# mataiyuan/ASD-SLAM

Hardware: AMD Instinct MI355X
Metric: frames/sec end-to-end tracking+LocalBA, KITTI 00 mono @2000 keypoints (higher is better)
Workload: dtype f32

## Files before the change

asd-slam_amd/csrc/asdnet.hip:

```cpp
#include "ctx.h"

#include <algorithm>
#include <cmath>
#include <cstring>

typedef float f32x16 __attribute__((ext_vector_type(16)));
typedef float f32x4 __attribute__((ext_vector_type(4)));


namespace {

struct LayerSpec { int cout, cin, k, stride, pad; };
const LayerSpec kLayers[7] = {{32, 1, 3, 1, 1},   {32, 32, 3, 1, 1},   {64, 32, 3, 2, 1},  {64, 64, 3, 1, 1},
                              {128, 64, 3, 2, 1}, {128, 128, 3, 1, 1}, {128, 128, 8, 1, 0}};

template <int CIN, int COUT, int HIN, int S, int ROWS, int WM, int WN, int KC, int PP = 1, int RING = 2>
struct ConvCfg {
  static constexpr int HO = HIN / S;
  static constexpr int INROWS = (ROWS - 1) * S + 3;
  static constexpr int INCOLS = (HO - 1) * S + 3;
  static constexpr int CPAD = CIN + 4;
  static constexpr int NW = WM * WN;
  static constexpr int NTH = 64 * NW;
  static constexpr int M_PATCH = ROWS * HO;
// ... 352 lines not shown
    cur ^= 1;
  }
#undef LOAD_TILE
#undef STORE_TILE
}

#define ASD_X3_PD 2
#ifndef ASD_X3_RB
#define ASD_X3_RB 3
#endif
typedef __bf16 bf16x8 __attribute__((ext_vector_type(8)));
typedef uint32_t u32x4 __attribute__((ext_vector_type(4)));

template <int CIN, int COUT, int HIN, int S, int ROWS, int WM, int WN, int PP = 1, int NP = 3>
struct X3Cfg {
  static constexpr int HO = HIN / S;
  static constexpr int INROWS = (ROWS - 1) * S + 3;
  static constexpr int INCOLS = (HO - 1) * S + 3;
  static constexpr int PIXB = CIN * 2 * NP + 16;
  static constexpr int GRPB = 16 * NP;
  static constexpr bool PLANAR = NP == 2 && S == 2;
  static constexpr int GSTR = PLANAR ? 16 : GRPB;
  static constexpr int PSTR = PLANAR ? CIN * 2 : 16;
  static constexpr int NW = WM * WN;
  static constexpr int NTH = 64 * NW;
  static constexpr int M_PATCH = ROWS * HO;
  static constexpr int M_WG = PP * M_PATCH;
  static constexpr int MT = M_WG / 32 / WM;
  static constexpr int NT = COUT / 32 / WN;
  static constexpr int KCH = 32;
// ... 70 lines not shown
  for (int k = 0; k < 4; ++k) asm volatile("" : "+v"(x[k]));
  float sum = (x[0] + x[1]) + (x[2] + x[3]);
  for (int off = 32; off >= 1; off >>= 1) sum += __shfl_xor(sum, off);
  if (lane == 0) red[wave] = sum;
  asd_syncthreads();
  const float mean = ((red[0] + red[1]) + (red[2] + red[3])) * (1.0f / 1024.0f);
  float d[4], ss = 0.f;
  for (int k = 0; k < 4; ++k) { d[k] = x[k] - mean; ss += d[k] * d[k]; }
  for (int off = 32; off >= 1; off >>= 1) ss += __shfl_xor(ss, off);
  if (lane == 0) red[4 + wave] = ss;
  asd_syncthreads();
  const float sd = sqrtf(((red[4] + red[5]) + (red[6] + red[7])) * (1.0f / 1023.0f)) + 1e-7f;
  if (t == 0) { stats[2 * (size_t)patch] = mean; stats[2 * (size_t)patch + 1] = sd; }
}

template <int CIN, int COUT, int HIN, int S, int ROWS, int WM, int WN, int PP, bool FUSE1 = false, int NP = 3, bool PAIR = false>
__device__ __forceinline__ void conv_x3_tile(const int bid, const void* __restrict__ in_, const uint8_t* __restrict__ wimg,
                                                         const float* __restrict__ bias, float* __restrict__ out,
                                                         const float* __restrict__ w1, const float* __restrict__ b1, int n,
                                                         unsigned long long* __restrict__ stamps, float in_scale, float out_scale,
                                                         const float* __restrict__ stats = nullptr) {
  using C = X3Cfg<CIN, COUT, HIN, S, ROWS, WM, WN, PP, NP>;
  constexpr int NTH = C::NTH, MT = C::MT, NCW = C::NCW;
  static_assert(!PAIR || NP == 2, "the pair format belongs to the two-piece form");
  extern __shared__ __attribute__((aligned(16))) uint8_t smem_b[];
  int t = threadIdx.x;
  asm volatile("" : "+v"(t));
  const int lane = t & 63, wave = t >> 6;
  const int wm = wave / WN, wn = wave % WN;
  constexpr int BANDS = C::HO / ROWS;
  const int patch = (bid / BANDS) * PP, band = bid % BANDS;
  const int r0 = band * ROWS;
  unsigned long long st_t0 = 0, st_t1 = 0;
  if (stamps) st_t0 = st_t1 = __builtin_amdgcn_s_memtime();
#define X3_STAMP(k) do { if (stamps && t == 0) stamps[16 * bid + (k)] = __builtin_amdgcn_s_memtime() - st_t0; } while (0)

  constexpr int SUB = 2, KG = C::KCH / 8, TW = 32 / SUB;
  const int kg = lane >> 4, lr = lane & 15;
  const uint8_t* wl = wimg + ((size_t)kg * COUT + wn * NCW + lr) * 16;
  constexpr int NB = NCW / TW;
  auto load_b = [&](int c, u32x4 (&b)[NB][NP]) {
    const uint8_t* wc = wl + (size_t)c * C::CHUNKB;
#pragma unroll
    for (int nb = 0; nb < NB; ++nb)
#pragma unroll
      for (int p = 0; p < NP; ++p) b[nb][p] = *reinterpret_cast<const u32x4*>(wc + (size_t)p * KG * COUT * 16 + nb * TW * 16);
  };
  constexpr int RB = C::NCHUNK % ASD_X3_RB == 0 ? ASD_X3_RB : 3;
  static_assert(C::NCHUNK % RB == 0, "chunk count");
  u32x4 br[RB][NB][NP];
#pragma unroll
  for (int d = 0; d < RB - 1; ++d) load_b(d, br[d]);

  if constexpr (FUSE1) {
    static_assert(!FUSE1 || (CIN == 32 && HIN == 32 && S == 1 && PP == 1 && (C::NW == 4 || C::NW == 8)), "conv1 fusion is for conv2 only");
    float* pin = reinterpret_cast<float*>(smem_b + C::ACT_BYTES);
    float* wsh = pin + (ROWS + 4) * 36;
    float* red = wsh + 320;
    const uint8_t* patches = static_cast<const uint8_t*>(in_);
    for (int i = t; i < (ROWS + 4) * 36; i += NTH) {
      const int j = i / 36, c = i % 36, y = r0 - 2 + j;
      if (!(c >= 1 && c <= 32 && y >= 0 && y < 32)) pin[i] = 0.f;
    }
    for (int i = t; i < 288; i += NTH) wsh[i] = w1[i];
    if (t < 32) wsh[288 + t] = b1[t];
    const bool ld = C::NW == 4 || wave < 4;
    const uchar4 v = ld ? reinterpret_cast<const uchar4*>(patches + (size_t)patch * 1024)[t] : make_uchar4(0, 0, 0, 0);
// ... 17 lines not shown
      float ss = 0.f;
      for (int k = 0; k < 4; ++k) { d[k] = x[k] - mean; ss += d[k] * d[k]; }
      for (int off = 32; off >= 1; off >>= 1) ss += __shfl_xor(ss, off);
      if (lane == 0 && ld) red[4 + wave] = ss;
      asd_syncthreads();
      sd = sqrtf(((red[4] + red[5]) + (red[6] + red[7])) * (1.0f / 1023.0f)) + 1e-7f;
    }
    if (ld) {
      const int idx = t * 4, y = idx >> 5, x0 = idx & 31;
      const int j = y - (r0 - 2);
      if (j >= 0 && j < ROWS + 4)
        for (int k = 0; k < 4; ++k) pin[j * 36 + x0 + k + 1] = d[k] / sd;
    }
    asd_syncthreads();
    if (stamps) st_t1 = __builtin_amdgcn_s_memtime();
    constexpr int NPIX = C::INROWS * C::INCOLS;
    const int q = t & 3;
    float wq[8][9], bq1[8];
#pragma unroll
    for (int c = 0; c < 8; ++c) {
      bq1[c] = wsh[288 + 8 * q + c];
#pragma unroll
      for (int k = 0; k < 9; ++k) wq[c][k] = wsh[(8 * q + c) * 9 + k];
    }
    for (int item = t; item < NPIX * 4; item += NTH) {
      const int pix = item >> 2;
      const int i = pix % C::INCOLS, j = pix / C::INCOLS;
      const int oy = r0 - 1 + j, ox = i - 1;
      f32x4 ra = {0.f, 0.f, 0.f, 0.f}, rb = {0.f, 0.f, 0.f, 0.f};
      if (oy >= 0 && oy < 32 && ox >= 0 && ox < 32) {
        float a[9];
#pragma unroll
        for (int ky = 0; ky < 3; ++ky)
#pragma unroll
          for (int kx = 0; kx < 3; ++kx) a[ky * 3 + kx] = pin[(j + ky) * 36 + ox + kx];
#pragma unroll
        for (int c = 0; c < 8; ++c) {
          float acc1 = bq1[c];
#pragma unroll
          for (int k = 0; k < 9; ++k) acc1 += a[k] * wq[c][k];
          const float r = acc1 > 0.f ? acc1 : 0.f;
          if (c < 4) ra[c] = r; else rb[c - 4] = r;
        }
      }
      u32x4 ph, pm, pl;
      uint8_t* dst = smem_b + pix * C::PIXB + q * C::GSTR;
      if constexpr (NP == 2) {
        split8_f16(ra, rb, in_scale, ph, pl);
        *reinterpret_cast<u32x4*>(dst) = ph;
        *reinterpret_cast<u32x4*>(dst + C::PSTR) = pl;
      } else {
        split8(ra, rb, ph, pm, pl);
        *reinterpret_cast<u32x4*>(dst) = ph;
        *reinterpret_cast<u32x4*>(dst + 16) = pm;
        *reinterpret_cast<u32x4*>(dst + 32) = pl;
      }
    }
  } else if constexpr (PAIR) {
    const uint8_t* inb = static_cast<const uint8_t*>(in_) + (size_t)patch * HIN * HIN * CIN * 4;
    constexpr int C8 = CIN / 8;
    constexpr int NPIXB = C::INROWS * C::INCOLS;
    static_assert(NTH % C8 == 0, "a thread keeps its channel group");
    constexpr int PSTEP = NTH / C8;
    constexpr int NROUND = (PP * NPIXB + PSTEP - 1) / PSTEP;
    constexpr int SBATCH = 8;
    const int c8 = t % C8, pix0 = t / C8;
    for (int rb = 0; rb < NROUND; rb += SBATCH) {
      u32x4 v0[SBATCH], v1[SBATCH];
#pragma unroll
      for (int b = 0; b < SBATCH; ++b) {
        const int pixg = pix0 + (rb + b) * PSTEP;
        const int pp = pixg / NPIXB, pix = pixg % NPIXB;
// ... 53 lines not shown
            *reinterpret_cast<u32x4*>(dst + C::PSTR) = pl;
          } else {
            split8(v0[b], v1[b], ph, pm, pl);
            *reinterpret_cast<u32x4*>(dst) = ph;
            *reinterpret_cast<u32x4*>(dst + 16) = pm;
            *reinterpret_cast<u32x4*>(dst + 32) = pl;
          }
        }
      }
    }
  }
  X3_STAMP(12);
  asd_syncthreads();
  X3_STAMP(13);

  constexpr int NA = MT * SUB, AR = 4;
  typedef float accv __attribute__((ext_vector_type(4)));
  accv acc[NA][NB];
  for (int ma = 0; ma < NA; ++ma)
    for (int nb = 0; nb < NB; ++nb)
      for (int r = 0; r < AR; ++r) acc[ma][nb][r] = 0.f;
  auto tile_pixel = [&](int sg, int r16) -> int {
    if constexpr (NP == 2) {
      if constexpr (S == 1 && C::HO >= 16) return sg * 16 + (r16 < 4 ? 2 * r16 : r16 < 12 ? 2 * r16 - 7 : 2 * r16 - 16);
      else if constexpr (S == 2 && C::HO >= 16) return sg * 16 + r16;
      else if constexpr (S == 2) return sg * 16 + (r16 < 4 ? r16 : r16 < 12 ? r16 + 4 : r16 - 8);
      else {
        static_assert(S == 2 || C::HO >= 16 || (PP == 1 && C::HO == 8 && ROWS == 8), "eight rows x two columns per sub-tile");
        const int j = r16 < 4 ? r16 : r16 < 12 ? r16 - 4 : r16 - 8;
        return j * C::HO + 2 * sg + (r16 >= 4 && r16 < 12 ? 1 : 0);
      }
    } else return sg * TW + r16;
  };
  int abase[NA];
  for (int ma = 0; ma < NA; ++ma) {
    const int m = tile_pixel((wm * MT * 32 + ma * TW) / TW, lr);
    const int pp = PP > 1 ? m / C::M_PATCH : 0, mm = m - pp * C::M_PATCH;
    const int rr = mm / C::HO, ox = mm % C::HO;
    abase[ma] = pp * C::ACT_BYTES + ((rr * S) * C::INCOLS + ox * S) * C::PIXB + kg * C::GSTR;
  }
  auto chunk_off = [&](int c) {
    const int tap = c / C::NC16, c16 = c % C::NC16;
    return ((tap / 3) * C::INCOLS + (tap % 3)) * C::PIXB + c16 * (KG * C::GSTR);
  };
  auto load_a = [&](int off, u32x4 (&a)[NP]) {
#pragma unroll
    for (int p = 0; p < NP; ++p) a[p] = *reinterpret_cast<const u32x4*>(smem_b + off + p * C::PSTR);
  };
  auto bf = [](const u32x4& v) { return __builtin_bit_cast(bf16x8, v); };
  auto hf = [](const u32x4& v) { return __builtin_bit_cast(f16x8, v); };
  auto mma = [&](const u32x4& x, const u32x4& y, accv& c) {
    if constexpr (PAIR) c = __builtin_amdgcn_mfma_f32_16x16x32_f16(hf(y), hf(x), c, 0, 0, 0);
    else if constexpr (NP == 2) c = __builtin_amdgcn_mfma_f32_16x16x32_f16(hf(x), hf(y), c, 0, 0, 0);
    else c = __builtin_amdgcn_mfma_f32_16x16x32_bf16(bf(x), bf(y), c, 0, 0, 0);
  };

  constexpr int PD = ASD_X3_PD, RS = PD + 1;
  static_assert((RB * NA) % RS == 0, "ring slots must be static");
  u32x4 ar[RS][NP];
#pragma unroll
  for (int q = 0; q < PD; ++q) load_a(abase[q % NA] + chunk_off(q / NA), ar[q]);
  unsigned long long st_c = 0, st_r = 0;
  if (stamps) { st_c = __builtin_amdgcn_s_memtime(); st_r = __builtin_amdgcn_s_memrealtime(); }
  for (int c0 = 0; c0 < C::NCHUNK; c0 += RB) {
    int offs[RB + PD / NA + 2];
#pragma unroll
    for (int u = 0; u < RB + PD / NA + 2; ++u) offs[u] = chunk_off(c0 + u < C::NCHUNK ? c0 + u : C::NCHUNK - 1);
#pragma unroll
    for (int u = 0; u < RB; ++u) {
      const int c = c0 + u;
      load_b(c + RB - 1 < C::NCHUNK ? c + RB - 1 : C::NCHUNK - 1, br[(u + RB - 1) % RB]);
      __builtin_amdgcn_sched_group_barrier(0x020, NP * NB, 0);
      const u32x4 (&bc)[NB][NP] = br[u];
#pragma unroll
      for (int ma = 0; ma < NA; ++ma) {
        const int q = u * NA + ma;
        const int qn = q + PD;
        load_a(abase[qn % NA] + offs[qn / NA], ar[qn % RS]);
        const u32x4 (&ac)[NP] = ar[q % RS];
#pragma unroll
        for (int nb = 0; nb < NB; ++nb) {
          if constexpr (NP == 2) {
            mma(ac[1], bc[nb][0], acc[ma][nb]);
            mma(ac[0], bc[nb][1], acc[ma][nb]);
            mma(ac[0], bc[nb][0], acc[ma][nb]);
          } else {
            mma(ac[2], bc[nb][0], acc[ma][nb]);
            mma(ac[0], bc[nb][2], acc[ma][nb]);
            mma(ac[1], bc[nb][1], acc[ma][nb]);
            mma(ac[1], bc[nb][0], acc[ma][nb]);
            mma(ac[0], bc[nb][1], acc[ma][nb]);
            mma(ac[0], bc[nb][0], acc[ma][nb]);
          }
        }
#pragma unroll
        for (int p = 0; p < NP; ++p) {
          __builtin_amdgcn_sched_group_barrier(0x008, (NP * (NP + 1) / 2) * NB / NP, 0);
          __builtin_amdgcn_sched_group_barrier(0x100, 1, 0);
        }
      }
    }
  }

  if (stamps) {
    asm volatile("s_nop 0" ::"v"(acc[NA - 1][NB - 1][0]));
    const unsigned long long e_c = __builtin_amdgcn_s_memtime(), e_r = __builtin_amdgcn_s_memrealtime();
    if (t == 0) { stamps[16 * bid] = e_c - st_c; stamps[16 * bid + 1] = e_r - st_r; stamps[16 * bid + 2] = st_t1 - st_t0; stamps[16 * bid + 3] = st_c - st_t1; stamps[16 * bid + 6] = st_t0; }
  }
  if constexpr (PAIR) {
    uint8_t* opb = reinterpret_cast<uint8_t*>(out) + ((size_t)patch * C::HO + r0) * C::HO * COUT * 4;
    for (int nb = 0; nb < NB; ++nb) {
      const int co0 = wn * NCW + nb * TW + 4 * kg;
      const f32x4 bv = *reinterpret_cast<const f32x4*>(bias + co0);
      for (int ma = 0; ma < NA; ++ma) {
        const int m0 = wm * MT * 32 + ma * TW;
        const int pp = PP > 1 ? m0 / C::M_PATCH : 0;
        if (PP > 1 && patch + pp >= n) continue;
        const int m = tile_pixel(m0 / TW, lr);
        float v[4];
#pragma unroll
        for (int r = 0; r < 4; ++r) { const float x = acc[ma][nb][r] * out_scale + bv[r]; v[r] = x < 0.f ? 0.f : x; }
        uint32_t hh[2], ll[2];
        split4_mix(v[0], v[1], v[2], v[3], kActScale, hh, ll);
        const auto s0 = __builtin_amdgcn_permlane16_swap(hh[0], ll[0], false, false);
        const auto s1 = __builtin_amdgcn_permlane16_swap(hh[1], ll[1], false, false);
        uint8_t* o = opb + ((size_t)pp * C::HO * C::HO + (size_t)(m - pp * C::M_PATCH)) * COUT * 4 + (co0 >> 3) * 32 + (kg & 1) * 16;
        *reinterpret_cast<u32x4*>(o) = u32x4{s0[0], s1[0], s0[1], s1[1]};
      }
    }
  } else {
  float* op = out + ((size_t)patch * C::HO + r0) * C::HO * COUT;
  for (int nb = 0; nb < NB; ++nb) {
    const int co = wn * NCW + nb * TW + lr;
    const float bv = bias[co];
    for (int ma = 0; ma < NA; ++ma) {
      const int m0 = wm * MT * 32 + ma * TW;
      const int pp = PP > 1 ? m0 / C::M_PATCH : 0;
      if (PP > 1 && patch + pp >= n) continue;
      for (int r = 0; r < AR; ++r) {
        const int m = tile_pixel(m0 / TW, 4 * kg + r);
        const size_t o = (size_t)pp * C::HO * C::HO * COUT + (size_t)(m - pp * C::M_PATCH) * COUT + co;
        const float v = (NP == 2 ? acc[ma][nb][r] * out_scale : acc[ma][nb][r]) + bv;
// ... 283 lines not shown
#define L2S_CFG 32, 32, 32, 1, 8, ASD_L2_WMN, 1
#ifndef ASD_L3_ROWS
#define ASD_L3_ROWS 4
#endif
#define L3S_CFG 32, 64, 32, 2, ASD_L3_ROWS, ASD_L3_WMN, 1
#define L4S_CFG 64, 64, 16, 1, 8, ASD_L4_WMN, 1
#ifndef ASD_L5_RWMN
#define ASD_L5_RWMN 8, 1, 4
#endif
#ifndef ASD_L6_WMN
#define ASD_L6_WMN 1, 4
#endif
#define L5S_CFG 64, 128, 16, 2, ASD_L5_RWMN, 1
#define L6S_CFG 128, 128, 8, 1, 8, ASD_L6_WMN, 1

template <int CIN, int COUT, int HIN, int S, int ROWS, int WM, int WN, int KC, int PP = 1, int RING = 2, bool FUSE1 = false>
hipError_t launch_conv(hipStream_t st, const void* in, const float* wimg, const float* bias, float* out, int n,
                       const float* w1 = nullptr, const float* b1 = nullptr) {
  using C = ConvCfg<CIN, COUT, HIN, S, ROWS, WM, WN, KC, PP, RING>;
  auto kern = k_conv_mfma<CIN, COUT, HIN, S, ROWS, WM, WN, KC, PP, RING, FUSE1>;
  constexpr int lds = C::LDS_BYTES + (FUSE1 ? ((ROWS + 4) * 36 + 320 + 8) * 4 : 0);
  static_assert(lds <= 160 * 1024, "band + weight ring do not fit LDS");
  static AsdPerDeviceOnce attr_set;
  int dev_ = 0;
  (void)hipGetDevice(&dev_);
  if (attr_set.need(dev_)) {
    hipError_t e = hipFuncSetAttribute(reinterpret_cast<const void*>(kern), hipFuncAttributeMaxDynamicSharedMemorySize, lds);
    if (e != hipSuccess) return e;
    attr_set.done(dev_);
  }
// ... 34 lines not shown
  static AsdPerDeviceOnce attr_set;
  int dev_ = 0;
  (void)hipGetDevice(&dev_);
  if (attr_set.need(dev_)) {
    hipError_t e = hipFuncSetAttribute(reinterpret_cast<const void*>(kern), hipFuncAttributeMaxDynamicSharedMemorySize, lds);
    if (e != hipSuccess) return e;
    attr_set.done(dev_);
  }
  const int ntiles = ((n + PP - 1) / PP) * (C::HO / ROWS);
  if (grid_out) *grid_out = ntiles;
  hipLaunchKernelGGL(kern, dim3(ntiles), dim3(C::NTH), lds, st, in, static_cast<const uint8_t*>(wimg), bias, out, w1, b1, n, stamps,
                     in_scale, out_scale, stats);
  return hipGetLastError();
}

inline void split3_host(float x, uint16_t& h, uint16_t& m, uint16_t& l) {
  uint32_t u, r1u, r2u;
  memcpy(&u, &x, 4);
  const uint32_t hu = u & 0xffff0000u;
  float hf; memcpy(&hf, &hu, 4);
  const float r1 = x - hf;
  memcpy(&r1u, &r1, 4);
  const uint32_t mu = r1u & 0xffff0000u;
  float mf; memcpy(&mf, &mu, 4);
  const float r2 = r1 - mf;
  memcpy(&r2u, &r2, 4);
  h = (uint16_t)(hu >> 16); m = (uint16_t)(mu >> 16); l = (uint16_t)(r2u >> 16);
}

inline void split2_host(float xs, uint16_t& h, uint16_t& l) {
// ... 41 lines not shown
}

}

int asdnet_alloc(asd_ctx* ctx) {
  const size_t np = (size_t)ctx->cfg.max_patches;
  const size_t npad = (np + 31) / 32 * 32;
  ASD_HIP_CHECK(ctx, hipMalloc(&ctx->d_act[0], np * 32768 * sizeof(float)));
  ASD_HIP_CHECK(ctx, hipMalloc(&ctx->d_act[1], np * 32768 * sizeof(float)));
  ASD_HIP_CHECK(ctx, hipMalloc(&ctx->d_part, (size_t)FC_SK * npad * 128 * sizeof(float)));
  ASD_HIP_CHECK(ctx, hipMalloc(&ctx->d_patches, np * 1024));
  ASD_HIP_CHECK(ctx, hipMalloc(&ctx->d_desc, np * 128 * sizeof(float)));
  ASD_HIP_CHECK(ctx, hipHostMalloc(reinterpret_cast<void**>(&ctx->h_range), 64));
  *ctx->h_range = 0;
  if (const char* e = getenv("ASD_ASDNET_PAIR")) ctx->net_pair = atoi(e) != 0;
  return ASD_OK;
}

void asdnet_free(asd_ctx* ctx) {
  for (int i = 0; i < 2; ++i) if (ctx->d_act[i]) (void)hipFree(ctx->d_act[i]);
  if (ctx->d_part) (void)hipFree(ctx->d_part);
  if (ctx->d_patches) (void)hipFree(ctx->d_patches);
  if (ctx->d_desc) (void)hipFree(ctx->d_desc);
  if (ctx->h_range) (void)hipHostFree(ctx->h_range);
  if (ctx->d_w1) (void)hipFree(ctx->d_w1);
  for (int i = 0; i < 7; ++i) {
    if (ctx->d_bias[i]) (void)hipFree(ctx->d_bias[i]);
    if (ctx->d_wimg[i]) (void)hipFree(ctx->d_wimg[i]);
    if (ctx->d_wx3[i]) (void)hipFree(ctx->d_wx3[i]);
    if (ctx->d_wx2[i]) (void)hipFree(ctx->d_wx2[i]);
// ... 98 lines not shown
  PROF_MARK(0);
  PROF_MARK(1);
#define CALIB(l, buf, elems) do { if (ctx->d_calib) { hipLaunchKernelGGL(k_absmax, dim3(256), dim3(256), 0, st, buf, (size_t)n * (elems), ctx->d_calib + (l)); ASD_HIP_CHECK(ctx, hipGetLastError()); } } while (0)
  ctx->d_act6 = a1;
  if (ctx->net_split) {
    const bool p2 = ctx->net_pieces == 2;
    const bool pair = p2 && ctx->net_pair && !ctx->d_calib;
    const float* x3_stats = nullptr;
#define X3_LAUNCH(CFG, FUSE, l, src, dst, w1p, b1p)                                                                                       \
  (pair ? launch_conv_x3<CFG, FUSE, 2, true>(st, src, ctx->d_wx2[l], ctx->d_bias[l], dst, n, w1p, b1p, nullptr, nullptr, kActScale,          \
                                     1.f / (kActScale * ctx->wx2_scale[l]), x3_stats)                                                               \
   : p2 ? launch_conv_x3<CFG, FUSE, 2>(st, src, ctx->d_wx2[l], ctx->d_bias[l], dst, n, w1p, b1p, nullptr, nullptr, kActScale,               \
                                     1.f / (kActScale * ctx->wx2_scale[l]), x3_stats)                                                               \
      : launch_conv_x3<CFG, FUSE, 3>(st, src, ctx->d_wx3[l], ctx->d_bias[l], dst, n, w1p, b1p, nullptr, nullptr, 1.f, 1.f,                \
                                     x3_stats))
    hipLaunchKernelGGL(k_patch_stats, dim3(n), dim3(256), 0, st, d_patches, ctx->d_part, n);
    ASD_HIP_CHECK(ctx, hipGetLastError());
    x3_stats = ctx->d_part;
    ASD_HIP_CHECK(ctx, (X3_LAUNCH(L2S_CFG, true, 1, d_patches, a1, ctx->d_w1, ctx->d_bias[0])));
    x3_stats = nullptr;
    CALIB(1, a1, 32 * 32 * 32);
    PROF_MARK(2);
    ASD_HIP_CHECK(ctx, (X3_LAUNCH(L3S_CFG, false, 2, a1, a0, nullptr, nullptr)));
    CALIB(2, a0, 16 * 16 * 64);
    PROF_MARK(3);
    ASD_HIP_CHECK(ctx, (X3_LAUNCH(L4S_CFG, false, 3, a0, a1, nullptr, nullptr)));
    CALIB(3, a1, 16 * 16 * 64);
    PROF_MARK(4);
    ASD_HIP_CHECK(ctx, (X3_LAUNCH(L5S_CFG, false, 4, a1, a0, nullptr, nullptr)));
    CALIB(4, a0, 8 * 8 * 128);
    PROF_MARK(5);
    ASD_HIP_CHECK(ctx, (X3_LAUNCH(L6S_CFG, false, 5, a0, a1, nullptr, nullptr)));
#undef X3_LAUNCH
    CALIB(5, a1, 8 * 8 * 128);
    PROF_MARK(6);
    if (pair)
      hipLaunchKernelGGL(k_fc_x2, dim3((npad + FCS_MP - 1) / FCS_MP, FC_SK), dim3(256), 0, st, reinterpret_cast<const uint8_t*>(a1),
                         static_cast<const uint8_t*>(ctx->d_wx2[6]), ctx->d_part, n, npad, 1.f / (kActScale * ctx->wx2_scale[6]));
    else
      hipLaunchKernelGGL(k_fc_x3, dim3((npad + FCS_MP - 1) / FCS_MP, FC_SK), dim3(256), 0, st, a1, static_cast<const uint8_t*>(ctx->d_wx3[6]), ctx->d_part, n, npad);
// ... 200 lines not shown
```

asd-slam_amd/csrc/ctx.h:

```cpp
#pragma once
#include <hip/hip_runtime.h>

#include <atomic>
#include <cstdarg>
#include <cstdio>
#include <cstdlib>
#include <cstring>
#include <functional>
#include <mutex>
#include <string>
#include <vector>

#include "../../include/asd_slam.h"

#define ASD_HIP_CHECK(ctx, expr)                                                          \
  do {                                                                                    \
    hipError_t _e = (expr);                                                               \
    if (_e != hipSuccess) {                                                               \
      (ctx)->set_error("%s failed: %s (%s:%d)", #expr, hipGetErrorString(_e), __FILE__, __LINE__); \
      return ASD_ERR_HIP;                                                                 \
    }                                                                                     \
  } while (0)

struct AsdPerDeviceOnce {
// ... 213 lines not shown
  bool match_replay_host = false;
  bool ba_struct_host = false;
  int gba_solve = 0;
  bool gba_update_fma = false;
  void* d_wx2[7] = {};
  float wx2_scale[7] = {1, 1, 1, 1, 1, 1, 1};
  int net_pieces_req = 2;
  int net_pieces = 2;
  int net_split = 0x3f;
  float* d_act[2] = {};
  float* d_part = nullptr;
  int* h_range = nullptr;
  std::string calib_note;
  unsigned* d_calib = nullptr;
  bool net_pair = true;
  float* d_act6 = nullptr;
  uint8_t* d_patches = nullptr;
  int patches_n = 0;
  float* d_desc = nullptr;
  bool keep_pyramid = false;
  const uint8_t* d_pyr_view = nullptr;
  AsdDevBuf stereo_scratch;
  float* d_desc_last = nullptr;
  hipEvent_t ev_adopt = nullptr;
  bool adopt_pending = false;

  struct FrontendState* fe = nullptr;
  UndistortMap* und = nullptr;
  int last_n = 0;

// ... 122 lines not shown
```

Measured before the change: 1300.

## Fuse conv2 and conv3 of descriptor net into one per-patch kernel

Measured after the change: 1294, median of 2. No clear change (-0.5%).

```diff
diff --git a/asd-slam_amd/csrc/asdnet.hip b/asd-slam_amd/csrc/asdnet.hip
--- a/asd-slam_amd/csrc/asdnet.hip
+++ b/asd-slam_amd/csrc/asdnet.hip
@@ -390,6 +390,7 @@
 
 template <int CIN, int COUT, int HIN, int S, int ROWS, int WM, int WN, int PP = 1, int NP = 3>
 struct X3Cfg {
+  static constexpr int STRIDE = S, BROWS = ROWS, NPATCH = PP, PIECES = NP, NCOUT = COUT;
   static constexpr int HO = HIN / S;
   static constexpr int INROWS = (ROWS - 1) * S + 3;
   static constexpr int INCOLS = (HO - 1) * S + 3;
@@ -490,6 +491,170 @@
   if (t == 0) { stats[2 * (size_t)patch] = mean; stats[2 * (size_t)patch + 1] = sd; }
 }
 
+
+template <class C>
+__device__ __forceinline__ int x3_tile_pixel(int sg, int r16) {
+  constexpr int S = C::STRIDE;
+  if constexpr (C::PIECES == 2) {
+    if constexpr (S == 1 && C::HO >= 16) return sg * 16 + (r16 < 4 ? 2 * r16 : r16 < 12 ? 2 * r16 - 7 : 2 * r16 - 16);
+    else if constexpr (S == 2 && C::HO >= 16) return sg * 16 + r16;
+    else if constexpr (S == 2) return sg * 16 + (r16 < 4 ? r16 : r16 < 12 ? r16 + 4 : r16 - 8);
+    else {
+      static_assert(S == 2 || C::HO >= 16 || (C::NPATCH == 1 && C::HO == 8 && C::BROWS == 8), "eight rows x two columns per sub-tile");
+      const int j = r16 < 4 ? r16 : r16 < 12 ? r16 - 4 : r16 - 8;
+      return j * C::HO + 2 * sg + (r16 >= 4 && r16 < 12 ? 1 : 0);
+    }
+  } else return sg * 16 + r16;
+}
+
+template <class C>
+__device__ __forceinline__ void x3_conv1_band(uint8_t* smem_b, const float* pin, const float* wsh, int r0, int t, float in_scale) {
+  constexpr int NPIX = C::INROWS * C::INCOLS, NP = C::PIECES;
+  const int q = t & 3;
+  float wq[8][9], bq1[8];
+#pragma unroll
+  for (int c = 0; c < 8; ++c) {
+    bq1[c] = wsh[288 + 8 * q + c];
+#pragma unroll
+    for (int k = 0; k < 9; ++k) wq[c][k] = wsh[(8 * q + c) * 9 + k];
+  }
+  for (int item = t; item < NPIX * 4; item += C::NTH) {
+    const int pix = item >> 2;
+    const int i = pix % C::INCOLS, j = pix / C::INCOLS;
+    const int oy = r0 - 1 + j, ox = i - 1;
+    f32x4 ra = {0.f, 0.f, 0.f, 0.f}, rb = {0.f, 0.f, 0.f, 0.f};
+    if (oy >= 0 && oy < 32 && ox >= 0 && ox < 32) {
+      float a[9];
+#pragma unroll
+      for (int ky = 0; ky < 3; ++ky)
+#pragma unroll
+        for (int kx = 0; kx < 3; ++kx) a[ky * 3 + kx] = pin[(j + ky) * 36 + ox + kx];
+#pragma unroll
+      for (int c = 0; c < 8; ++c) {
+        float acc1 = bq1[c];
+#pragma unroll
+        for (int k = 0; k < 9; ++k) acc1 += a[k] * wq[c][k];
+        const float r = acc1 > 0.f ? acc1 : 0.f;
+        if (c < 4) ra[c] = r; else rb[c - 4] = r;
+      }
+    }
+    u32x4 ph, pm, pl;
+    uint8_t* dst = smem_b + pix * C::PIXB + q * C::GSTR;
+    if constexpr (NP == 2) {
+      split8_f16(ra, rb, in_scale, ph, pl);
+      *reinterpret_cast<u32x4*>(dst) = ph;
+      *reinterpret_cast<u32x4*>(dst + C::PSTR) = pl;
+    } else {
+      split8(ra, rb, ph, pm, pl);
+      *reinterpret_cast<u32x4*>(dst) = ph;
+      *reinterpret_cast<u32x4*>(dst + 16) = pm;
+      *reinterpret_cast<u32x4*>(dst + 32) = pl;
+    }
+  }
+}
+
+template <class C, bool PAIR>
+struct X3Mma {
+  static constexpr int NP = C::PIECES, COUT = C::NCOUT;
+  static constexpr int SUB = 2, KG = C::KCH / 8, TW = 32 / SUB;
+  static constexpr int NB = C::NCW / TW;
+  static constexpr int NA = C::MT * SUB;
+  static constexpr int RB = C::NCHUNK % ASD_X3_RB == 0 ? ASD_X3_RB : 3;
+  static_assert(C::NCHUNK % RB == 0, "chunk count");
+  static constexpr int PD = ASD_X3_PD, RS = PD + 1;
+  static_assert((RB * NA) % RS == 0, "ring slots must be static");
+  typedef float accv __attribute__((ext_vector_type(4)));
+
+  const uint8_t* wl;
+  u32x4 br[RB][NB][NP];
+
+  __device__ __forceinline__ void load_b(int c, u32x4 (&b)[NB][NP]) const {
+    const uint8_t* wc = wl + (size_t)c * C::CHUNKB;
+#pragma unroll
+    for (int nb = 0; nb < NB; ++nb)
+#pragma unroll
+      for (int p = 0; p < NP; ++p) b[nb][p] = *reinterpret_cast<const u32x4*>(wc + (size_t)p * KG * COUT * 16 + nb * TW * 16);
+  }
+  __device__ __forceinline__ void start(const uint8_t* __restrict__ wimg, int kg, int wn, int lr) {
+    wl = wimg + ((size_t)kg * COUT + wn * C::NCW + lr) * 16;
+#pragma unroll
+    for (int d = 0; d < RB - 1; ++d) load_b(d, br[d]);
+  }
+  static __device__ __forceinline__ int chunk_off(int c) {
+    const int tap = c / C::NC16, c16 = c % C::NC16;
+    return ((tap / 3) * C::INCOLS + (tap % 3)) * C::PIXB + c16 * (KG * C::GSTR);
+  }
+  static __device__ __forceinline__ void load_a(const uint8_t* smem, int off, u32x4 (&a)[NP]) {
+#pragma unroll
+    for (int p = 0; p < NP; ++p) a[p] = *reinterpret_cast<const u32x4*>(smem + off + p * C::PSTR);
+  }
+  static __device__ __forceinline__ void mma(const u32x4& x, const u32x4& y, accv& c) {
+    if constexpr (PAIR) c = __builtin_amdgcn_mfma_f32_16x16x32_f16(__builtin_bit_cast(f16x8, y), __builtin_bit_cast(f16x8, x), c, 0, 0, 0);
+    else if constexpr (NP == 2) c = __builtin_amdgcn_mfma_f32_16x16x32_f16(__builtin_bit_cast(f16x8, x), __builtin_bit_cast(f16x8, y), c, 0, 0, 0);
+    else c = __builtin_amdgcn_mfma_f32_16x16x32_bf16(__builtin_bit_cast(bf16x8, x), __builtin_bit_cast(bf16x8, y), c, 0, 0, 0);
+  }
+  __device__ __forceinline__ void run(const uint8_t* smem, const int (&abase)[NA], accv (&acc)[NA][NB], bool stamped, unsigned long long& st_c,
+                                      unsigned long long& st_r) {
+    for (int ma = 0; ma < NA; ++ma)
+      for (int nb = 0; nb < NB; ++nb)
+        for (int r = 0; r < 4; ++r) acc[ma][nb][r] = 0.f;
+    u32x4 ar[RS][NP];
+#pragma unroll
+    for (int q = 0; q < PD; ++q) load_a(smem, abase[q % NA] + chunk_off(q / NA), ar[q]);
+    if (stamped) { st_c = __builtin_amdgcn_s_memtime(); st_r = __builtin_amdgcn_s_memrealtime(); }
+    for (int c0 = 0; c0 < C::NCHUNK; c0 += RB) {
+      int offs[RB + PD / NA + 2];
+#pragma unroll
+      for (int u = 0; u < RB + PD / NA + 2; ++u) offs[u] = chunk_off(c0 + u < C::NCHUNK ? c0 + u : C::NCHUNK - 1);
+#pragma unroll
+      for (int u = 0; u < RB; ++u) {
+        const int c = c0 + u;
+        load_b(c + RB - 1 < C::NCHUNK ? c + RB - 1 : C::NCHUNK - 1, br[(u + RB - 1) % RB]);
+        __builtin_amdgcn_sched_group_barrier(0x020, NP * NB, 0);
+        const u32x4 (&bc)[NB][NP] = br[u];
+#pragma unroll
+        for (int ma = 0; ma < NA; ++ma) {
+          const int q = u * NA + ma;
+          const int qn = q + PD;
+          load_a(smem, abase[qn % NA] + offs[qn / NA], ar[qn % RS]);
+          const u32x4 (&ac)[NP] = ar[q % RS];
+#pragma unroll
+          for (int nb = 0; nb < NB; ++nb) {
+            if constexpr (NP == 2) {
+              mma(ac[1], bc[nb][0], acc[ma][nb]);
+              mma(ac[0], bc[nb][1], acc[ma][nb]);
+              mma(ac[0], bc[nb][0], acc[ma][nb]);
+            } else {
+              mma(ac[2], bc[nb][0], acc[ma][nb]);
+              mma(ac[0], bc[nb][2], acc[ma][nb]);
+              mma(ac[1], bc[nb][1], acc[ma][nb]);
+              mma(ac[1], bc[nb][0], acc[ma][nb]);
+              mma(ac[0], bc[nb][1], acc[ma][nb]);
+              mma(ac[0], bc[nb][0], acc[ma][nb]);
+            }
+          }
+#pragma unroll
+          for (int p = 0; p < NP; ++p) {
+            __builtin_amdgcn_sched_group_barrier(0x008, (NP * (NP + 1) / 2) * NB / NP, 0);
+            __builtin_amdgcn_sched_group_barrier(0x100, 1, 0);
+          }
+        }
+      }
+    }
+  }
+};
+
+__device__ __forceinline__ u32x4 x3_pair_value(const f32x4& a, const f32x4& bv, float out_scale) {
+  float v[4];
+#pragma unroll
+  for (int r = 0; r < 4; ++r) { const float x = a[r] * out_scale + bv[r]; v[r] = x < 0.f ? 0.f : x; }
+  uint32_t hh[2], ll[2];
+  split4_mix(v[0], v[1], v[2], v[3], kActScale, hh, ll);
+  const auto s0 = __builtin_amdgcn_permlane16_swap(hh[0], ll[0], false, false);
+  const auto s1 = __builtin_amdgcn_permlane16_swap(hh[1], ll[1], false, false);
+  return u32x4{s0[0], s1[0], s0[1], s1[1]};
+}
+
 template <int CIN, int COUT, int HIN, int S, int ROWS, int WM, int WN, int PP, bool FUSE1 = false, int NP = 3, bool PAIR = false>
 __device__ __forceinline__ void conv_x3_tile(const int bid, const void* __restrict__ in_, const uint8_t* __restrict__ wimg,
                                                          const float* __restrict__ bias, float* __restrict__ out,
@@ -511,22 +676,11 @@
   if (stamps) st_t0 = st_t1 = __builtin_amdgcn_s_memtime();
 #define X3_STAMP(k) do { if (stamps && t == 0) stamps[16 * bid + (k)] = __builtin_amdgcn_s_memtime() - st_t0; } while (0)
 
-  constexpr int SUB = 2, KG = C::KCH / 8, TW = 32 / SUB;
+  using M = X3Mma<C, PAIR>;
+  constexpr int TW = M::TW, NB = M::NB;
   const int kg = lane >> 4, lr = lane & 15;
-  const uint8_t* wl = wimg + ((size_t)kg * COUT + wn * NCW + lr) * 16;
-  constexpr int NB = NCW / TW;
-  auto load_b = [&](int c, u32x4 (&b)[NB][NP]) {
-    const uint8_t* wc = wl + (size_t)c * C::CHUNKB;
-#pragma unroll
-    for (int nb = 0; nb < NB; ++nb)
-#pragma unroll
-      for (int p = 0; p < NP; ++p) b[nb][p] = *reinterpret_cast<const u32x4*>(wc + (size_t)p * KG * COUT * 16 + nb * TW * 16);
-  };
-  constexpr int RB = C::NCHUNK % ASD_X3_RB == 0 ? ASD_X3_RB : 3;
-  static_assert(C::NCHUNK % RB == 0, "chunk count");
-  u32x4 br[RB][NB][NP];
-#pragma unroll
-  for (int d = 0; d < RB - 1; ++d) load_b(d, br[d]);
+  M mfma;
+  mfma.start(wimg, kg, wn, lr);
 
   if constexpr (FUSE1) {
     static_assert(!FUSE1 || (CIN == 32 && HIN == 32 && S == 1 && PP == 1 && (C::NW == 4 || C::NW == 8)), "conv1 fusion is for conv2 only");
@@ -574,48 +728,7 @@
     }
     asd_syncthreads();
     if (stamps) st_t1 = __builtin_amdgcn_s_memtime();
-    constexpr int NPIX = C::INROWS * C::INCOLS;
-    const int q = t & 3;
-    float wq[8][9], bq1[8];
-#pragma unroll
-    for (int c = 0; c < 8; ++c) {
-      bq1[c] = wsh[288 + 8 * q + c];
-#pragma unroll
-      for (int k = 0; k < 9; ++k) wq[c][k] = wsh[(8 * q + c) * 9 + k];
-    }
-    for (int item = t; item < NPIX * 4; item += NTH) {
-      const int pix = item >> 2;
-      const int i = pix % C::INCOLS, j = pix / C::INCOLS;
-      const int oy = r0 - 1 + j, ox = i - 1;
-      f32x4 ra = {0.f, 0.f, 0.f, 0.f}, rb = {0.f, 0.f, 0.f, 0.f};
-      if (oy >= 0 && oy < 32 && ox >= 0 && ox < 32) {
-        float a[9];
-#pragma unroll
-        for (int ky = 0; ky < 3; ++ky)
-#pragma unroll
-          for (int kx = 0; kx < 3; ++kx) a[ky * 3 + kx] = pin[(j + ky) * 36 + ox + kx];
-#pragma unroll
-        for (int c = 0; c < 8; ++c) {
-          float acc1 = bq1[c];
-#pragma unroll
-          for (int k = 0; k < 9; ++k) acc1 += a[k] * wq[c][k];
-          const float r = acc1 > 0.f ? acc1 : 0.f;
-          if (c < 4) ra[c] = r; else rb[c - 4] = r;
-        }
-      }
-      u32x4 ph, pm, pl;
-      uint8_t* dst = smem_b + pix * C::PIXB + q * C::GSTR;
-      if constexpr (NP == 2) {
-        split8_f16(ra, rb, in_scale, ph, pl);
-        *reinterpret_cast<u32x4*>(dst) = ph;
-        *reinterpret_cast<u32x4*>(dst + C::PSTR) = pl;
-      } else {
-        split8(ra, rb, ph, pm, pl);
-        *reinterpret_cast<u32x4*>(dst) = ph;
-        *reinterpret_cast<u32x4*>(dst + 16) = pm;
-        *reinterpret_cast<u32x4*>(dst + 32) = pl;
-      }
-    }
+    x3_conv1_band<C>(smem_b, pin, wsh, r0, t, in_scale);
   } else if constexpr (PAIR) {
     const uint8_t* inb = static_cast<const uint8_t*>(in_) + (size_t)patch * HIN * HIN * CIN * 4;
     constexpr int C8 = CIN / 8;
@@ -699,24 +812,9 @@
   asd_syncthreads();
   X3_STAMP(13);
 
-  constexpr int NA = MT * SUB, AR = 4;
-  typedef float accv __attribute__((ext_vector_type(4)));
-  accv acc[NA][NB];
-  for (int ma = 0; ma < NA; ++ma)
-    for (int nb = 0; nb < NB; ++nb)
-      for (int r = 0; r < AR; ++r) acc[ma][nb][r] = 0.f;
-  auto tile_pixel = [&](int sg, int r16) -> int {
-    if constexpr (NP == 2) {
-      if constexpr (S == 1 && C::HO >= 16) return sg * 16 + (r16 < 4 ? 2 * r16 : r16 < 12 ? 2 * r16 - 7 : 2 * r16 - 16);
-      else if constexpr (S == 2 && C::HO >= 16) return sg * 16 + r16;
-      else if constexpr (S == 2) return sg * 16 + (r16 < 4 ? r16 : r16 < 12 ? r16 + 4 : r16 - 8);
-      else {
-        static_assert(S == 2 || C::HO >= 16 || (PP == 1 && C::HO == 8 && ROWS == 8), "eight rows x two columns per sub-tile");
-        const int j = r16 < 4 ? r16 : r16 < 12 ? r16 - 4 : r16 - 8;
-        return j * C::HO + 2 * sg + (r16 >= 4 && r16 < 12 ? 1 : 0);
-      }
-    } else return sg * TW + r16;
-  };
+  constexpr int NA = M::NA, AR = 4;
+  typename M::accv acc[NA][NB];
+  auto tile_pixel = [](int sg, int r16) -> int { return x3_tile_pixel<C>(sg, r16); };
   int abase[NA];
   for (int ma = 0; ma < NA; ++ma) {
     const int m = tile_pixel((wm * MT * 32 + ma * TW) / TW, lr);
@@ -724,68 +822,8 @@
     const int rr = mm / C::HO, ox = mm % C::HO;
     abase[ma] = pp * C::ACT_BYTES + ((rr * S) * C::INCOLS + ox * S) * C::PIXB + kg * C::GSTR;
   }
-  auto chunk_off = [&](int c) {
-    const int tap = c / C::NC16, c16 = c % C::NC16;
-    return ((tap / 3) * C::INCOLS + (tap % 3)) * C::PIXB + c16 * (KG * C::GSTR);
-  };
-  auto load_a = [&](int off, u32x4 (&a)[NP]) {
-#pragma unroll
-    for (int p = 0; p < NP; ++p) a[p] = *reinterpret_cast<const u32x4*>(smem_b + off + p * C::PSTR);
-  };
-  auto bf = [](const u32x4& v) { return __builtin_bit_cast(bf16x8, v); };
-  auto hf = [](const u32x4& v) { return __builtin_bit_cast(f16x8, v); };
-  auto mma = [&](const u32x4& x, const u32x4& y, accv& c) {
-    if constexpr (PAIR) c = __builtin_amdgcn_mfma_f32_16x16x32_f16(hf(y), hf(x), c, 0, 0, 0);
-    else if constexpr (NP == 2) c = __builtin_amdgcn_mfma_f32_16x16x32_f16(hf(x), hf(y), c, 0, 0, 0);
-    else c = __builtin_amdgcn_mfma_f32_16x16x32_bf16(bf(x), bf(y), c, 0, 0, 0);
-  };
-
-  constexpr int PD = ASD_X3_PD, RS = PD + 1;
-  static_assert((RB * NA) % RS == 0, "ring slots must be static");
-  u32x4 ar[RS][NP];
-#pragma unroll
-  for (int q = 0; q < PD; ++q) load_a(abase[q % NA] + chunk_off(q / NA), ar[q]);
   unsigned long long st_c = 0, st_r = 0;
-  if (stamps) { st_c = __builtin_amdgcn_s_memtime(); st_r = __builtin_amdgcn_s_memrealtime(); }
-  for (int c0 = 0; c0 < C::NCHUNK; c0 += RB) {
-    int offs[RB + PD / NA + 2];
-#pragma unroll
-    for (int u = 0; u < RB + PD / NA + 2; ++u) offs[u] = chunk_off(c0 + u < C::NCHUNK ? c0 + u : C::NCHUNK - 1);
-#pragma unroll
-    for (int u = 0; u < RB; ++u) {
-      const int c = c0 + u;
-      load_b(c + RB - 1 < C::NCHUNK ? c + RB - 1 : C::NCHUNK - 1, br[(u + RB - 1) % RB]);
-      __builtin_amdgcn_sched_group_barrier(0x020, NP * NB, 0);
-      const u32x4 (&bc)[NB][NP] = br[u];
-#pragma unroll
-      for (int ma = 0; ma < NA; ++ma) {
-        const int q = u * NA + ma;
-        const int qn = q + PD;
-        load_a(abase[qn % NA] + offs[qn / NA], ar[qn % RS]);
-        const u32x4 (&ac)[NP] = ar[q % RS];
-#pragma unroll
-        for (int nb = 0; nb < NB; ++nb) {
-          if constexpr (NP == 2) {
-            mma(ac[1], bc[nb][0], acc[ma][nb]);
-            mma(ac[0], bc[nb][1], acc[ma][nb]);
-            mma(ac[0], bc[nb][0], acc[ma][nb]);
-          } else {
-            mma(ac[2], bc[nb][0], acc[ma][nb]);
-            mma(ac[0], bc[nb][2], acc[ma][nb]);
-            mma(ac[1], bc[nb][1], acc[ma][nb]);
-            mma(ac[1], bc[nb][0], acc[ma][nb]);
-            mma(ac[0], bc[nb][1], acc[ma][nb]);
-            mma(ac[0], bc[nb][0], acc[ma][nb]);
-          }
-        }
-#pragma unroll
-        for (int p = 0; p < NP; ++p) {
-          __builtin_amdgcn_sched_group_barrier(0x008, (NP * (NP + 1) / 2) * NB / NP, 0);
-          __builtin_amdgcn_sched_group_barrier(0x100, 1, 0);
-        }
-      }
-    }
-  }
+  mfma.run(smem_b, abase, acc, stamps != nullptr, st_c, st_r);
 
   if (stamps) {
     asm volatile("s_nop 0" ::"v"(acc[NA - 1][NB - 1][0]));
@@ -802,15 +840,8 @@
         const int pp = PP > 1 ? m0 / C::M_PATCH : 0;
         if (PP > 1 && patch + pp >= n) continue;
         const int m = tile_pixel(m0 / TW, lr);
-        float v[4];
-#pragma unroll
-        for (int r = 0; r < 4; ++r) { const float x = acc[ma][nb][r] * out_scale + bv[r]; v[r] = x < 0.f ? 0.f : x; }
-        uint32_t hh[2], ll[2];
-        split4_mix(v[0], v[1], v[2], v[3], kActScale, hh, ll);
-        const auto s0 = __builtin_amdgcn_permlane16_swap(hh[0], ll[0], false, false);
-        const auto s1 = __builtin_amdgcn_permlane16_swap(hh[1], ll[1], false, false);
         uint8_t* o = opb + ((size_t)pp * C::HO * C::HO + (size_t)(m - pp * C::M_PATCH)) * COUT * 4 + (co0 >> 3) * 32 + (kg & 1) * 16;
-        *reinterpret_cast<u32x4*>(o) = u32x4{s0[0], s1[0], s0[1], s1[1]};
+        *reinterpret_cast<u32x4*>(o) = x3_pair_value(acc[ma][nb], bv, out_scale);
       }
     }
   } else {
@@ -1124,6 +1155,150 @@
 #define L5S_CFG 64, 128, 16, 2, ASD_L5_RWMN, 1
 #define L6S_CFG 128, 128, 8, 1, 8, ASD_L6_WMN, 1
 
+struct Fuse23 {
+  using C2 = X3Cfg<L2S_CFG, 2>;
+  using C3 = X3Cfg<L3S_CFG, 2>;
+  static constexpr int GROUPS = C3::HO / C3::BROWS;
+  static constexpr int PIN_FLOATS = (C2::BROWS + 4) * 36;
+  static constexpr int LDS_BYTES = C2::ACT_BYTES + (PIN_FLOATS + 320 + 8) * 4;
+  static constexpr int ROW_SLOTS = C3::INCOLS * (C3::PIXB / 16 - 1);
+  static_assert(C2::NTH == 256 && C3::NTH == 256 && C2::NPATCH == 1 && C3::NPATCH == 1, "one workgroup of four waves per patch");
+  static_assert(C2::NCOUT == 32 && C2::HO / C2::BROWS == GROUPS && C2::BROWS == 2 * C3::BROWS, "a conv2 band feeds exactly one conv3 band");
+  static_assert(C3::PLANAR && C3::INROWS == C2::BROWS + 1 && C3::INCOLS == C2::HO + 1 && C3::PIXB == 144, "conv3's band: one carried row + the new ones, one pad column");
+  static_assert(C3::ACT_BYTES <= C2::ACT_BYTES, "conv3's band lies inside the dead conv1 band");
+  static_assert(ROW_SLOTS <= 2 * 256, "the carried row: at most two slots per thread");
+  static_assert(LDS_BYTES <= 163840 / 3, "three workgroups per CU");
+};
+
+__global__ __launch_bounds__(256, 3) void k_conv_x3_fuse23(const uint8_t* __restrict__ patches, const uint8_t* __restrict__ w2img,
+                                                            const float* __restrict__ bias2, const uint8_t* __restrict__ w3img,
+                                                            const float* __restrict__ bias3, uint8_t* __restrict__ out,
+                                                            const float* __restrict__ w1, const float* __restrict__ b1, float in_scale,
+                                                            float out_scale2, float out_scale3) {
+  using F = Fuse23;
+  using C2 = F::C2;
+  using C3 = F::C3;
+  using M2 = X3Mma<C2, true>;
+  using M3 = X3Mma<C3, true>;
+  extern __shared__ __attribute__((aligned(16))) uint8_t smem_b[];
+  float* pin = reinterpret_cast<float*>(smem_b + C2::ACT_BYTES);
+  float* wsh = pin + F::PIN_FLOATS;
+  float* red = wsh + 320;
+  const int patch = blockIdx.x;
+  unsigned long long st_none = 0;
+
+  float dn[4];
+  {
+    const int t = threadIdx.x, lane = t & 63, wave = t >> 6;
+    for (int i = t; i < 288; i += 256) wsh[i] = w1[i];
+    if (t < 32) wsh[288 + t] = b1[t];
+    const uchar4 v = reinterpret_cast<const uchar4*>(patches + (size_t)patch * 1024)[t];
+    const float inv255 = (float)(1.0 / 255);
+    float x[4] = {v.x * inv255, v.y * inv255, v.z * inv255, v.w * inv255};
+#pragma unroll
+    for (int k = 0; k < 4; ++k) asm volatile("" : "+v"(x[k]));
+    float sum = (x[0] + x[1]) + (x[2] + x[3]);
+    for (int off = 32; off >= 1; off >>= 1) sum += __shfl_xor(sum, off);
+    if (lane == 0) red[wave] = sum;
+    asd_syncthreads();
+    const float mean = ((red[0] + red[1]) + (red[2] + red[3])) * (1.0f / 1024.0f);
+    float d[4], ss = 0.f;
+    for (int k = 0; k < 4; ++k) { d[k] = x[k] - mean; ss += d[k] * d[k]; }
+    for (int off = 32; off >= 1; off >>= 1) ss += __shfl_xor(ss, off);
+    if (lane == 0) red[4 + wave] = ss;
+    asd_syncthreads();
+    const float sd = sqrtf(((red[4] + red[5]) + (red[6] + red[7])) * (1.0f / 1023.0f)) + 1e-7f;
+    for (int k = 0; k < 4; ++k) dn[k] = d[k] / sd;
+  }
+  auto fill_pin = [&](int r0, int t) {
+    for (int i = t; i < F::PIN_FLOATS; i += 256) {
+      const int j = i / 36, c = i % 36, y = r0 - 2 + j;
+      if (!(c >= 1 && c <= 32 && y >= 0 && y < 32)) pin[i] = 0.f;
+    }
+    const int idx = t * 4, y = idx >> 5, x0 = idx & 31;
+    const int j = y - (r0 - 2);
+    if (j >= 0 && j < C2::BROWS + 4)
+      for (int k = 0; k < 4; ++k) pin[j * 36 + x0 + k + 1] = dn[k];
+  };
+  fill_pin(0, threadIdx.x);
+  asd_syncthreads();
+
+  u32x4 carry[2] = {u32x4{0, 0, 0, 0}, u32x4{0, 0, 0, 0}};
+#pragma unroll 1
+  for (int g = 0; g < F::GROUPS; ++g) {
+    int t = threadIdx.x;
+    asm volatile("" : "+v"(t));
+    const int lane = t & 63, wave = t >> 6, kg = lane >> 4, lr = lane & 15;
+    constexpr int TW = M2::TW;
+
+    M2 m2;
+    m2.start(w2img, kg, 0, lr);
+    x3_conv1_band<C2>(smem_b, pin, wsh, g * C2::BROWS, t, in_scale);
+    asd_syncthreads();
+
+    typename M2::accv acc2[M2::NA][M2::NB];
+    {
+      int abase[M2::NA];
+      for (int ma = 0; ma < M2::NA; ++ma) {
+        const int m = x3_tile_pixel<C2>((wave * C2::MT * 32 + ma * TW) / TW, lr);
+        const int rr = m / C2::HO, ox = m % C2::HO;
+        abase[ma] = (rr * C2::INCOLS + ox) * C2::PIXB + kg * C2::GSTR;
+      }
+      m2.run(smem_b, abase, acc2, false, st_none, st_none);
+    }
+    M3 m3;
+    m3.start(w3img, kg, wave, lr);
+    asd_syncthreads();
+
+    for (int nb = 0; nb < M2::NB; ++nb) {
+      const int co0 = nb * TW + 4 * kg;
+      const f32x4 bv = *reinterpret_cast<const f32x4*>(bias2 + co0);
+      for (int ma = 0; ma < M2::NA; ++ma) {
+        const int m = x3_tile_pixel<C2>((wave * C2::MT * 32 + ma * TW) / TW, lr);
+        const int rr = m / C2::HO, ox = m % C2::HO;
+        uint8_t* o = smem_b + ((rr + 1) * C3::INCOLS + ox + 1) * C3::PIXB + (co0 >> 3) * C3::GSTR + (kg & 1) * C3::PSTR;
+        *reinterpret_cast<u32x4*>(o) = x3_pair_value(acc2[ma][nb], bv, out_scale2);
+      }
+    }
+#pragma unroll
+    for (int k = 0; k < 2; ++k) {
+      const int s = t + 256 * k;
+      if (s < F::ROW_SLOTS) *reinterpret_cast<u32x4*>(smem_b + (s >> 3) * C3::PIXB + (s & 7) * 16) = carry[k];
+    }
+    if (t < 8 * C2::BROWS)
+      *reinterpret_cast<u32x4*>(smem_b + (1 + (t >> 3)) * C3::INCOLS * C3::PIXB + (t & 7) * 16) = u32x4{0, 0, 0, 0};
+    if (g + 1 < F::GROUPS) fill_pin((g + 1) * C2::BROWS, t);
+    asd_syncthreads();
+
+    typename M3::accv acc3[M3::NA][M3::NB];
+    {
+      int abase[M3::NA];
+      for (int ma = 0; ma < M3::NA; ++ma) {
+        const int m = x3_tile_pixel<C3>(ma, lr);
+        const int rr = m / C3::HO, ox = m % C3::HO;
+        abase[ma] = ((rr * 2) * C3::INCOLS + ox * 2) * C3::PIXB + kg * C3::GSTR;
+      }
+      m3.run(smem_b, abase, acc3, false, st_none, st_none);
+    }
+#pragma unroll
+    for (int k = 0; k < 2; ++k) {
+      const int s = t + 256 * k;
+      if (s < F::ROW_SLOTS) carry[k] = *reinterpret_cast<const u32x4*>(smem_b + (C2::BROWS * C3::INCOLS + (s >> 3)) * C3::PIXB + (s & 7) * 16);
+    }
+    {
+      uint8_t* opb = out + ((size_t)patch * C3::HO + g * C3::BROWS) * C3::HO * C3::NCOUT * 4;
+      const int co0 = wave * C3::NCW + 4 * kg;
+      const f32x4 bv = *reinterpret_cast<const f32x4*>(bias3 + co0);
+      for (int ma = 0; ma < M3::NA; ++ma) {
+        const int m = x3_tile_pixel<C3>(ma, lr);
+        uint8_t* o = opb + (size_t)m * C3::NCOUT * 4 + (co0 >> 3) * 32 + (kg & 1) * 16;
+        *reinterpret_cast<u32x4*>(o) = x3_pair_value(acc3[ma][0], bv, out_scale3);
+      }
+    }
+    asd_syncthreads();
+  }
+}
+
 template <int CIN, int COUT, int HIN, int S, int ROWS, int WM, int WN, int KC, int PP = 1, int RING = 2, bool FUSE1 = false>
 hipError_t launch_conv(hipStream_t st, const void* in, const float* wimg, const float* bias, float* out, int n,
                        const float* w1 = nullptr, const float* b1 = nullptr) {
@@ -1188,6 +1363,22 @@
   return hipGetLastError();
 }
 
+hipError_t launch_conv_x3_fuse23(hipStream_t st, const uint8_t* patches, const void* w2img, const float* bias2, const void* w3img, const float* bias3,
+                                 float* out, int n, const float* w1, const float* b1, float in_scale, float out_scale2, float out_scale3) {
+  constexpr int lds = Fuse23::LDS_BYTES;
+  static AsdPerDeviceOnce attr_set;
+  int dev_ = 0;
+  (void)hipGetDevice(&dev_);
+  if (attr_set.need(dev_)) {
+    hipError_t e = hipFuncSetAttribute(reinterpret_cast<const void*>(k_conv_x3_fuse23), hipFuncAttributeMaxDynamicSharedMemorySize, lds);
+    if (e != hipSuccess) return e;
+    attr_set.done(dev_);
+  }
+  hipLaunchKernelGGL(k_conv_x3_fuse23, dim3(n), dim3(256), lds, st, patches, static_cast<const uint8_t*>(w2img), bias2, static_cast<const uint8_t*>(w3img),
+                     bias3, reinterpret_cast<uint8_t*>(out), w1, b1, in_scale, out_scale2, out_scale3);
+  return hipGetLastError();
+}
+
 inline void split3_host(float x, uint16_t& h, uint16_t& m, uint16_t& l) {
   uint32_t u, r1u, r2u;
   memcpy(&u, &x, 4);
@@ -1259,6 +1450,7 @@
   ASD_HIP_CHECK(ctx, hipHostMalloc(reinterpret_cast<void**>(&ctx->h_range), 64));
   *ctx->h_range = 0;
   if (const char* e = getenv("ASD_ASDNET_PAIR")) ctx->net_pair = atoi(e) != 0;
+  if (const char* e = getenv("ASD_ASDNET_FUSE23")) ctx->net_fuse23 = atoi(e) != 0;
   return ASD_OK;
 }
 
@@ -1387,16 +1579,23 @@
                                      1.f / (kActScale * ctx->wx2_scale[l]), x3_stats)                                                               \
       : launch_conv_x3<CFG, FUSE, 3>(st, src, ctx->d_wx3[l], ctx->d_bias[l], dst, n, w1p, b1p, nullptr, nullptr, 1.f, 1.f,                \
                                      x3_stats))
-    hipLaunchKernelGGL(k_patch_stats, dim3(n), dim3(256), 0, st, d_patches, ctx->d_part, n);
-    ASD_HIP_CHECK(ctx, hipGetLastError());
-    x3_stats = ctx->d_part;
-    ASD_HIP_CHECK(ctx, (X3_LAUNCH(L2S_CFG, true, 1, d_patches, a1, ctx->d_w1, ctx->d_bias[0])));
-    x3_stats = nullptr;
-    CALIB(1, a1, 32 * 32 * 32);
-    PROF_MARK(2);
-    ASD_HIP_CHECK(ctx, (X3_LAUNCH(L3S_CFG, false, 2, a1, a0, nullptr, nullptr)));
-    CALIB(2, a0, 16 * 16 * 64);
-    PROF_MARK(3);
+    if (pair && ctx->net_fuse23) {
+      ASD_HIP_CHECK(ctx, launch_conv_x3_fuse23(st, d_patches, ctx->d_wx2[1], ctx->d_bias[1], ctx->d_wx2[2], ctx->d_bias[2], a0, n, ctx->d_w1, ctx->d_bias[0],
+                                               kActScale, 1.f / (kActScale * ctx->wx2_scale[1]), 1.f / (kActScale * ctx->wx2_scale[2])));
+      PROF_MARK(2);
+      PROF_MARK(3);
+    } else {
+      hipLaunchKernelGGL(k_patch_stats, dim3(n), dim3(256), 0, st, d_patches, ctx->d_part, n);
+      ASD_HIP_CHECK(ctx, hipGetLastError());
+      x3_stats = ctx->d_part;
+      ASD_HIP_CHECK(ctx, (X3_LAUNCH(L2S_CFG, true, 1, d_patches, a1, ctx->d_w1, ctx->d_bias[0])));
+      x3_stats = nullptr;
+      CALIB(1, a1, 32 * 32 * 32);
+      PROF_MARK(2);
+      ASD_HIP_CHECK(ctx, (X3_LAUNCH(L3S_CFG, false, 2, a1, a0, nullptr, nullptr)));
+      CALIB(2, a0, 16 * 16 * 64);
+      PROF_MARK(3);
+    }
     ASD_HIP_CHECK(ctx, (X3_LAUNCH(L4S_CFG, false, 3, a0, a1, nullptr, nullptr)));
     CALIB(3, a1, 16 * 16 * 64);
     PROF_MARK(4);
diff --git a/asd-slam_amd/csrc/ctx.h b/asd-slam_amd/csrc/ctx.h
--- a/asd-slam_amd/csrc/ctx.h
+++ b/asd-slam_amd/csrc/ctx.h
@@ -251,6 +251,7 @@
   std::string calib_note;
   unsigned* d_calib = nullptr;
   bool net_pair = true;
+  bool net_fuse23 = true;
   float* d_act6 = nullptr;
   uint8_t* d_patches = nullptr;
   int patches_n = 0;
```
